# NorthStarUAS/ImageAnalysis

Measured on AMD Instinct MI355X. Metric: image_pairs_matched_per_sec, higher is better.
Workload: dtype u8 (int8 MFMA, int32 accumulate)

## Files before the change

### imageanalysis_amd/csrc/match_knn2sym.hip

```cpp
#include "iamx_common.h"

namespace {

typedef int v4i __attribute__((ext_vector_type(4)));
typedef int v2i __attribute__((ext_vector_type(2)));
typedef int v16i __attribute__((ext_vector_type(16)));
typedef unsigned v2u __attribute__((ext_vector_type(2)));

#ifndef IAMX_DESC_OFFSET
#define IAMX_DESC_OFFSET 128
#endif
constexpr int D = IAMX_DESC_DIM;
constexpr int CHUNK = 128;
constexpr int BIG = 0x3F000000;

struct Pack3Args {
    const void *src;
    const int64_t *src_off;
    int64_t single_n;
    const int32_t *dst_off;
    int8_t *dst;
    int32_t *sn2, *sct, *sperm, *sinv;
    int32_t *n2, *nb, *pos;
    int n_img;
// ... 67 lines not shown
    for (int m = 32; m >= 1; m >>= 1) {
        lo = min(lo, __shfl_xor(lo, m));
        hi = max(hi, __shfl_xor(hi, m));
    }
    if (lane == 0) { atomicMin(&s_lo, lo); atomicMax(&s_hi, hi); }
    __syncthreads();
    lo = s_lo;
    int shift = 0;
    while (((int64_t)s_hi - lo) >> shift >= RANK_BINS) ++shift;
    for (int r = tid; r < n; r += 1024) atomicAdd(&cursor[(key[r] - lo) >> shift], 1);
    __syncthreads();
    int c[4], t = 0, mx = 0;
#pragma unroll
    for (int k = 0; k < 4; ++k) {
        c[k] = cursor[4 * tid + k];
        t += c[k];
        mx = max(mx, c[k]);
    }
    int x = t;
#pragma unroll
    for (int sft = 1; sft < 64; sft <<= 1) {
        const int y = __shfl_up(x, sft);
        if (lane >= sft) x += y;
    }
    if (lane == 63) wsum[wave] = x;
#pragma unroll
    for (int m = 32; m >= 1; m >>= 1) mx = max(mx, __shfl_xor(mx, m));
    if (lane == 0) atomicMax(&s_max, mx);
    __syncthreads();
    int woff = 0;
    for (int w = 0; w < wave; ++w) woff += wsum[w];
    int run = woff + x - t;
#pragma unroll
    for (int k = 0; k < 4; ++k) {
        start[4 * tid + k] = run;
        run += c[k];
    }
    if (tid == 1023) start[RANK_BINS] = run;
    __syncthreads();
    if (s_max > RANK_BIN_LIMIT) {
        if (tid == 0) P.sct[d0] = RANK_TODO;
        return;
    }
    if (tid == 0) P.sct[d0] = 0;
    for (int b = tid; b < RANK_BINS; b += 1024) cursor[b] = start[b];
    __syncthreads();
    for (int r = tid; r < n; r += 1024) {
        const int k = key[r];
        const int at = atomicAdd(&cursor[(k - lo) >> shift], 1);
        list_row[at] = r;
        list_key[at] = k;
    }
    __threadfence_block();
    __syncthreads();
    for (int r = tid; r < n; r += 1024) {
        const int k = key[r], b = (k - lo) >> shift;
        const int e = start[b + 1];
        int cnt = start[b];
        for (int i = start[b]; i < e; ++i) {
            const int kj = list_key[i], j = list_row[i];
            cnt += (kj < k) || (kj == k && j < r);
        }
        P.pos[r0 + r] = cnt;
    }
}

__global__ __launch_bounds__(256) void pack3_rank_kernel(Pack3Args P)
{
    __shared__ __attribute__((aligned(16))) int keys[1024];
    const int img = blockIdx.y;
    const int64_t r0 = P.src_off ? P.src_off[img] : 0;
    const int n = (int)(P.src_off ? P.src_off[img + 1] - r0 : P.single_n);
    if ((int)blockIdx.x * 256 >= n) return;
    if (P.sct[P.dst_off ? P.dst_off[img] : 0] != RANK_TODO) return;
    const int r = blockIdx.x * 256 + threadIdx.x;
    const int mine = r < n ? P.n2[r0 + r] : 0;
    const int tiles = (n + 1023) / 1024, per = (tiles + (int)gridDim.z - 1) / (int)gridDim.z;
    const int b_lo = (int)blockIdx.z * per * 1024, b_hi = min(n, b_lo + per * 1024);
    int cnt = 0;
    for (int base = b_lo; base < b_hi; base += 1024) {
        __syncthreads();
#pragma unroll
        for (int k = 0; k < 4; ++k) {
            const int j = base + k * 256 + threadIdx.x;
            keys[k * 256 + threadIdx.x] = j < n ? P.n2[r0 + j] : 0x7FFFFFFF;
        }
        __syncthreads();
        for (int j = 0; j < 1024; j += 4) {
            const v4i k = *reinterpret_cast<const v4i *>(&keys[j]);
            cnt += (k.x < mine) || (k.x == mine && base + j < r);
            cnt += (k.y < mine) || (k.y == mine && base + j + 1 < r);
            cnt += (k.z < mine) || (k.z == mine && base + j + 2 < r);
            cnt += (k.w < mine) || (k.w == mine && base + j + 3 < r);
        }
    }
    if (r < n) {
        if (gridDim.z == 1) P.pos[r0 + r] = cnt;
        else if (cnt) atomicAdd(&P.pos[r0 + r], cnt);
    }
}

template <typename SRC>
__global__ __launch_bounds__(256) void pack3_scatter_kernel(Pack3Args P)
{
    const int img = blockIdx.y;
    const int64_t r0 = P.src_off ? P.src_off[img] : 0;
    const int n = (int)(P.src_off ? P.src_off[img + 1] - r0 : P.single_n);
    const int d0 = P.dst_off ? P.dst_off[img] : 0;
    const int cap = (n + CHUNK - 1) / CHUNK * CHUNK;
    const int t = blockIdx.x * 256 + threadIdx.x;
    const int r = t >> 3, part = t & 7;
    if (r >= cap) return;
    if (r >= n) {
        *reinterpret_cast<uint4 *>(P.dst + (int64_t)(d0 + r) * D + part * 16) = make_uint4(0, 0, 0, 0);
        if (part == 0) {
            P.sn2[d0 + r] = 0;
            P.sct[d0 + r] = BIG;
            P.sperm[d0 + r] = -1;
            P.sinv[d0 + r] = -1;
        }
        return;
    }
    const SRC *p = static_cast<const SRC *>(P.src) + (r0 + r) * D + part * 16;
    unsigned w[4] = {0, 0, 0, 0};
#pragma unroll
    for (int i = 0; i < 16; ++i)
        w[i >> 2] |= (unsigned)((load_value(p, i) - IAMX_DESC_OFFSET) & 0xFF) << (8 * (i & 3));
    const int pos = d0 + P.pos[r0 + r];
    *reinterpret_cast<uint4 *>(P.dst + (int64_t)pos * D + part * 16) = make_uint4(w[0], w[1], w[2], w[3]);
    if (part == 0) {
        P.sn2[pos] = P.n2[r0 + r];
        P.sct[pos] = P.nb[r0 + r] >> 1;
        P.sperm[pos] = r;
        P.sinv[d0 + r] = pos - d0;
    }
}

constexpr int ROW_NO_BOUND = 0x7F000000;
__device__ __forceinline__ int pack_row_bounds(int L, int U1, int U2)
{
#if defined(IAMX_T_NOPACK)
    return U1;
#else
    typedef unsigned short us2 __attribute__((ext_vector_type(2)));
    const us2 d = __builtin_amdgcn_cvt_pk_u16((unsigned)(U1 - L), (unsigned)(U2 - L));
    return (int)__builtin_bit_cast(unsigned, d);
#endif
}
__device__ __forceinline__ void unpack_row_bounds(v2i e, int &L, int &U1, int &U2)
{
    const int d1 = e.y & 0xFFFF, d2 = (int)((unsigned)e.y >> 16);
    L = e.x;
    U1 = d1 == 0xFFFF ? ROW_NO_BOUND : e.x + d1;
    U2 = d2 == 0xFFFF ? ROW_NO_BOUND : e.x + d2;
}

struct SymArgs {
    const int8_t *sdesc;
    const int32_t *sn2, *sct;
    const int32_t *img_off, *img_n;
    const int32_t *upairs;
    const int32_t *wg_off;
    const int64_t *col_off;
    const int64_t *rowp_off;
    int32_t *col;
    int32_t *rowp;
    int n_u, total_wg;
    uint8_t *colmask;
};

__device__ __forceinline__ int uniform32(int x) { return __builtin_amdgcn_readfirstlane(x); }
__device__ __forceinline__ int64_t uniform64(int64_t x)
{
    return (int64_t)(((uint64_t)(unsigned)__builtin_amdgcn_readfirstlane((int)(x >> 32)) << 32) |
                     (unsigned)__builtin_amdgcn_readfirstlane((int)x));
}

template <bool FUSED>
__device__ __forceinline__ void half_wave_min16(int (&r)[16], int lo, int &m0, int &m1)
{
    int u[4], w[2];
    if constexpr (FUSED) {
        asm("s_nop 1\n\t"
            "v_min_i32_dpp %0, %0, %0 row_ror:8 row_mask:0xf bank_mask:0x3\n\t"
            "v_min_i32_dpp %0, %8, %8 row_ror:8 row_mask:0xf bank_mask:0xc\n\t"
            "v_min_i32_dpp %1, %1, %1 row_ror:8 row_mask:0xf bank_mask:0x3\n\t"
            "v_min_i32_dpp %1, %9, %9 row_ror:8 row_mask:0xf bank_mask:0xc\n\t"
            "v_min_i32_dpp %2, %2, %2 row_ror:8 row_mask:0xf bank_mask:0x3\n\t"
            "v_min_i32_dpp %2, %10, %10 row_ror:8 row_mask:0xf bank_mask:0xc\n\t"
            "v_min_i32_dpp %3, %3, %3 row_ror:8 row_mask:0xf bank_mask:0x3\n\t"
            "v_min_i32_dpp %3, %11, %11 row_ror:8 row_mask:0xf bank_mask:0xc\n\t"
            "v_min_i32_dpp %4, %4, %4 row_ror:8 row_mask:0xf bank_mask:0x3\n\t"
            "v_min_i32_dpp %4, %12, %12 row_ror:8 row_mask:0xf bank_mask:0xc\n\t"
            "v_min_i32_dpp %5, %5, %5 row_ror:8 row_mask:0xf bank_mask:0x3\n\t"
            "v_min_i32_dpp %5, %13, %13 row_ror:8 row_mask:0xf bank_mask:0xc\n\t"
            "v_min_i32_dpp %6, %6, %6 row_ror:8 row_mask:0xf bank_mask:0x3\n\t"
            "v_min_i32_dpp %6, %14, %14 row_ror:8 row_mask:0xf bank_mask:0xc\n\t"
            "v_min_i32_dpp %7, %7, %7 row_ror:8 row_mask:0xf bank_mask:0x3\n\t"
            "v_min_i32_dpp %7, %15, %15 row_ror:8 row_mask:0xf bank_mask:0xc"
            : "+v"(r[0]), "+v"(r[2]), "+v"(r[4]), "+v"(r[6]), "+v"(r[8]), "+v"(r[10]), "+v"(r[12]), "+v"(r[14])
            : "v"(r[1]), "v"(r[3]), "v"(r[5]), "v"(r[7]), "v"(r[9]), "v"(r[11]), "v"(r[13]), "v"(r[15]));
        asm("s_nop 1\n\t"
            "v_min_i32_dpp %0, %0, %0 row_ror:12 row_mask:0xf bank_mask:0x5\n\t"
            "v_min_i32_dpp %0, %4, %4 row_ror:4 row_mask:0xf bank_mask:0xa\n\t"
            "v_min_i32_dpp %1, %1, %1 row_ror:12 row_mask:0xf bank_mask:0x5\n\t"
            "v_min_i32_dpp %1, %5, %5 row_ror:4 row_mask:0xf bank_mask:0xa\n\t"
            "v_min_i32_dpp %2, %2, %2 row_ror:12 row_mask:0xf bank_mask:0x5\n\t"
            "v_min_i32_dpp %2, %6, %6 row_ror:4 row_mask:0xf bank_mask:0xa\n\t"
            "v_min_i32_dpp %3, %3, %3 row_ror:12 row_mask:0xf bank_mask:0x5\n\t"
            "v_min_i32_dpp %3, %7, %7 row_ror:4 row_mask:0xf bank_mask:0xa"
            : "+v"(r[0]), "+v"(r[4]), "+v"(r[8]), "+v"(r[12])
            : "v"(r[2]), "v"(r[6]), "v"(r[10]), "v"(r[14]));
#pragma unroll
        for (int k = 0; k < 4; ++k) u[k] = r[4 * k] + lo;
    } else {
        int s[8];
#pragma unroll
        for (int k = 0; k < 8; ++k) {
            const int a = r[2 * k], b = r[2 * k + 1];
            const int t1 = __builtin_amdgcn_update_dpp(b, a, 0x128, 0xF, 0x3, false);
            const int t2 = __builtin_amdgcn_update_dpp(a, b, 0x128, 0xF, 0xC, false);
            s[k] = min(t1, t2);
        }
#pragma unroll
        for (int k = 0; k < 4; ++k) {
            const int a = s[2 * k], b = s[2 * k + 1];
            const int t1 = __builtin_amdgcn_update_dpp(b, a, 0x12C, 0xF, 0x5, false);
            const int t2 = __builtin_amdgcn_update_dpp(a, b, 0x124, 0xF, 0xA, false);
            u[k] = min(t1, t2) + lo;
        }
    }
#pragma unroll
    for (int k = 0; k < 2; ++k) {
        const v2u x = __builtin_amdgcn_permlane16_swap((unsigned)u[2 * k], (unsigned)u[2 * k + 1], false, false);
        w[k] = min((int)x[0], (int)x[1]);
    }
#pragma unroll
    for (int k = 0; k < 2; ++k) {
        w[k] = min(w[k], __builtin_amdgcn_update_dpp(0, w[k], 0xB1, 0xF, 0xF, true));
        w[k] = min(w[k], __builtin_amdgcn_update_dpp(0, w[k], 0x4E, 0xF, 0xF, true));
    }
    m0 = w[0];
    m1 = w[1];
}

template <int P>
__device__ __forceinline__ void row_min16_piece(int (&r)[16], int (&u)[4], int lo, int *dst)
{
    if constexpr (P == 0) {
        asm("s_nop 1\n\t"
            "v_min_i32_dpp %0, %0, %0 row_ror:8 row_mask:0xf bank_mask:0x3\n\t"
            "v_min_i32_dpp %0, %4, %4 row_ror:8 row_mask:0xf bank_mask:0xc\n\t"
            "v_min_i32_dpp %1, %1, %1 row_ror:8 row_mask:0xf bank_mask:0x3\n\t"
            "v_min_i32_dpp %1, %5, %5 row_ror:8 row_mask:0xf bank_mask:0xc\n\t"
            "v_min_i32_dpp %2, %2, %2 row_ror:8 row_mask:0xf bank_mask:0x3\n\t"
            "v_min_i32_dpp %2, %6, %6 row_ror:8 row_mask:0xf bank_mask:0xc\n\t"
            "v_min_i32_dpp %3, %3, %3 row_ror:8 row_mask:0xf bank_mask:0x3\n\t"
            "v_min_i32_dpp %3, %7, %7 row_ror:8 row_mask:0xf bank_mask:0xc"
            : "+v"(r[0]), "+v"(r[2]), "+v"(r[4]), "+v"(r[6])
            : "v"(r[1]), "v"(r[3]), "v"(r[5]), "v"(r[7]));
    } else if constexpr (P == 1) {
        asm("s_nop 1\n\t"
            "v_min_i32_dpp %0, %0, %0 row_ror:8 row_mask:0xf bank_mask:0x3\n\t"
            "v_min_i32_dpp %0, %4, %4 row_ror:8 row_mask:0xf bank_mask:0xc\n\t"
            "v_min_i32_dpp %1, %1, %1 row_ror:8 row_mask:0xf bank_mask:0x3\n\t"
            "v_min_i32_dpp %1, %5, %5 row_ror:8 row_mask:0xf bank_mask:0xc\n\t"
            "v_min_i32_dpp %2, %2, %2 row_ror:8 row_mask:0xf bank_mask:0x3\n\t"
            "v_min_i32_dpp %2, %6, %6 row_ror:8 row_mask:0xf bank_mask:0xc\n\t"
            "v_min_i32_dpp %3, %3, %3 row_ror:8 row_mask:0xf bank_mask:0x3\n\t"
            "v_min_i32_dpp %3, %7, %7 row_ror:8 row_mask:0xf bank_mask:0xc"
            : "+v"(r[8]), "+v"(r[10]), "+v"(r[12]), "+v"(r[14])
            : "v"(r[9]), "v"(r[11]), "v"(r[13]), "v"(r[15]));
    } else if constexpr (P == 2) {
        asm("s_nop 1\n\t"
            "v_min_i32_dpp %0, %0, %0 row_ror:12 row_mask:0xf bank_mask:0x5\n\t"
            "v_min_i32_dpp %0, %4, %4 row_ror:4 row_mask:0xf bank_mask:0xa\n\t"
            "v_min_i32_dpp %1, %1, %1 row_ror:12 row_mask:0xf bank_mask:0x5\n\t"
            "v_min_i32_dpp %1, %5, %5 row_ror:4 row_mask:0xf bank_mask:0xa\n\t"
            "v_min_i32_dpp %2, %2, %2 row_ror:12 row_mask:0xf bank_mask:0x5\n\t"
            "v_min_i32_dpp %2, %6, %6 row_ror:4 row_mask:0xf bank_mask:0xa\n\t"
            "v_min_i32_dpp %3, %3, %3 row_ror:12 row_mask:0xf bank_mask:0x5\n\t"
            "v_min_i32_dpp %3, %7, %7 row_ror:4 row_mask:0xf bank_mask:0xa"
            : "+v"(r[0]), "+v"(r[4]), "+v"(r[8]), "+v"(r[12])
            : "v"(r[2]), "v"(r[6]), "v"(r[10]), "v"(r[14]));
#pragma unroll
        for (int k = 0; k < 4; ++k) u[k] = r[4 * k] + lo;
    } else {
        int w[2];
#pragma unroll
        for (int k = 0; k < 2; ++k) {
            const v2u x = __builtin_amdgcn_permlane16_swap((unsigned)u[2 * k], (unsigned)u[2 * k + 1], false, false);
            w[k] = min((int)x[0], (int)x[1]);
        }
#pragma unroll
        for (int k = 0; k < 2; ++k) {
            w[k] = min(w[k], __builtin_amdgcn_update_dpp(0, w[k], 0xB1, 0xF, 0xF, true));
            w[k] = min(w[k], __builtin_amdgcn_update_dpp(0, w[k], 0x4E, 0xF, 0xF, true));
        }
        dst[0] = w[0];
        dst[16] = w[1];
    }
}

template <int QW, int NW, int VARIANT, int PIPE, int MERGEW, int SLEEP, bool GROUPLO, int CH, int WPE>
__global__ __launch_bounds__(NW * 64, WPE) void knn2sym_kernel(SymArgs A)
{
    static_assert((VARIANT == 0 || VARIANT == 1) && PIPE > 0 && MERGEW == 2 && SLEEP == 0 && GROUPLO && CH == 128,
                  "only the shipped sweep is implemented");
    constexpr bool ITEMS = VARIANT == 1;
    constexpr int CHUNK = CH;
    constexpr int WGROWS = NW * QW * 32;
    constexpr int NT = NW * 64;
    constexpr int PIECES = CHUNK * D / 16 / NT;
    __shared__ __attribute__((aligned(16))) int8_t lds[2 * CHUNK * D + 2 * CHUNK * 4 + 3 * NW * CHUNK * 4 + 2 * NW * 4 + (2 * NW * CHUNK + NW * 256) * 4];
    int8_t *lds_tile = lds;
    int *lds_tb = reinterpret_cast<int *>(lds + 2 * CHUNK * D);
    int *lds_row = lds_tb + 2 * CHUNK;
    int *lds_cq = lds_row + 3 * NW * CHUNK;
    int *lds_dump = lds_cq + 2 * NW;
    const int tid = threadIdx.x, lane = tid & 63, wave = tid >> 6;
    const int c = lane & 31, g = lane >> 5;

    int vid;
    {
        const int total = A.total_wg, bid = blockIdx.x;
        const int xcd = bid & 7, k = bid >> 3, q = total >> 3, r = total & 7;
        vid = (xcd < r ? xcd * (q + 1) : r * (q + 1) + (xcd - r) * q) + k;
    }
    int lo = 0, hi = A.n_u;
    if constexpr (!ITEMS)
        while (hi - lo > 1) {
            const int mid = (lo + hi) >> 1;
            if (A.wg_off[mid] <= vid) lo = mid; else hi = mid;
        }
    int u = lo, u_end = 0, item_wgi = 0;
    if constexpr (ITEMS) {
        u = A.wg_off[3 * vid];
        u_end = u + A.wg_off[3 * vid + 1];
        item_wgi = A.wg_off[3 * vid + 2];
    }
    v4i bq[QW][4];
    int lo_lane;
    int bimg_held = -1;
    if constexpr (ITEMS) asm volatile("" : "+v"(u_end), "+v"(item_wgi), "+v"(bimg_held));
    int nx_b = 0, nx_a = 0, nx_boff = 0, nx_nb = 0, nx_aoff = 0, nx_na = 0;
    int64_t nx_rowp = 0;
    if constexpr (ITEMS) {
        nx_b = A.upairs[2 * u];
        nx_a = A.upairs[2 * u + 1];
        nx_boff = A.img_off[nx_b];
        nx_nb = A.img_n[nx_b];
        nx_aoff = A.img_off[nx_a];
        nx_na = A.img_n[nx_a];
        nx_rowp = A.rowp_off[u];
    }
    for (;;) {
        const int bimg = ITEMS ? uniform32(nx_b) : A.upairs[2 * u], aimg = ITEMS ? uniform32(nx_a) : A.upairs[2 * u + 1];
        const int boff = ITEMS ? uniform32(nx_boff) : A.img_off[bimg], nb = ITEMS ? uniform32(nx_nb) : A.img_n[bimg];
        const int aoff = ITEMS ? uniform32(nx_aoff) : A.img_off[aimg], na = ITEMS ? uniform32(nx_na) : A.img_n[aimg];
        const int capA = (na + CHUNK - 1) / CHUNK * CHUNK;
        const int nchunks = capA / CHUNK;
        const int wgi = ITEMS ? uniform32(item_wgi) : vid - A.wg_off[u];
        const int q0 = wgi * WGROWS + wave * (QW * 32);
        const bool wave_valid = q0 < nb;
        const int64_t rbase = (ITEMS ? uniform64(nx_rowp) : A.rowp_off[u]) + (int64_t)wgi * capA;
        if constexpr (ITEMS)
            if (uniform32(bimg_held) >= 0) __syncthreads();

        const int rc = (c & 16) | ((c & 3) << 2) | ((c >> 2) & 3);
        if (!ITEMS || bimg != uniform32(bimg_held)) {
            bimg_held = bimg;
#pragma unroll
            for (int qb = 0; qb < QW; ++qb) {
                int row = q0 + QW * rc + qb;
                row = row < nb ? row : nb - 1;
                const v4i *src = reinterpret_cast<const v4i *>(A.sdesc + (int64_t)(boff + row) * D);
#pragma unroll
                for (int s = 0; s < 4; ++s) {
                    bq[qb][s] = ~src[2 * s + g];
                    if constexpr (WPE == 1) asm volatile("" : "+a"(bq[qb][s]));
                }
            }
            lo_lane = 0;
            {
                int spread = 0;
                if (wave_valid) {
                    const int g_lo = rc & ~3, g_hi = rc | 3;
                    const int r_lo = q0 + QW * g_lo < nb ? q0 + QW * g_lo : nb - 1;
                    const int r_hi = q0 + QW * g_hi + QW - 1 < nb ? q0 + QW * g_hi + QW - 1 : nb - 1;
                    lo_lane = A.sn2[boff + r_lo] >> 1;
                    spread = (A.sn2[boff + r_hi] >> 1) - lo_lane;
                }
#pragma unroll
                for (int sh = 32; sh >= 1; sh >>= 1) spread = max(spread, __shfl_xor(spread, sh));
                if (lane == 0) lds_cq[wave] = spread;
            }
        }
        if (!wave_valid) {
#pragma unroll
            for (int k = 0; k < 3 * CHUNK / 64; ++k)
                lds_row[((k / (CHUNK / 64)) * NW + wave) * CHUNK + (k % (CHUNK / 64)) * 64 + lane] = BIG;
        }
        int m[QW][4];
#pragma unroll
        for (int qb = 0; qb < QW; ++qb)
#pragma unroll
            for (int k = 0; k < 4; ++k) m[qb][k] = BIG;

        const int8_t *tbase = A.sdesc + (int64_t)aoff * D;
        const int32_t *tci = A.sct + aoff;
        typedef __attribute__((address_space(3))) void *lds_ptr;
        auto stage_direct = [&](int ch, int buf) {
#pragma unroll
            for (int j = 0; j < PIECES; ++j) {
                const int e = j * NT + tid, row = e >> 3, slot = (e & 7) ^ ((row >> 1) & 7);
                const int8_t *gsrc = tbase + (int64_t)(ch * CHUNK + row) * D + slot * 16;
                int8_t *ldst = lds_tile + buf * (CHUNK * D) + (j * NT + wave * 64) * 16;
                __builtin_amdgcn_global_load_lds(gsrc, (lds_ptr)ldst, 16, 0, 0);
            }
            __builtin_amdgcn_global_load_lds(tci + ch * CHUNK + (tid & (CHUNK - 1)),
                                             (lds_ptr)(lds_tb + buf * CHUNK + (wave & (CHUNK / 64 - 1)) * 64), 4, 0, 0);
        };
        auto wait_direct = [&]() { __builtin_amdgcn_s_waitcnt(0x0F70); };
        constexpr int MROWS = CHUNK / MERGEW;
        static_assert(MROWS == 64 && NW % MERGEW == 0, "one merge row per lane");
        const int mrow = (wave % MERGEW) * MROWS + lane;
        const bool merger = wave < MERGEW;
        constexpr int RSRC_WORD3_DATA_FORMAT_32 = 4 << 15;
        constexpr int RANGE_DROP = 0x7FFFFFF0;
        const __amdgpu_buffer_rsrc_t rowp_rsrc =
            __builtin_amdgcn_make_buffer_rsrc(A.rowp + 2 * rbase, (short)0, capA * 8, RSRC_WORD3_DATA_FORMAT_32);
        int spread_w[NW];
        auto merge_rows = [&](int ch, int rbo, bool store) {
            int L = BIG, U1 = BIG, U2 = BIG;
#pragma unroll
            for (int w = 0; w < NW; ++w) {
                const int R = lds_row[rbo + w * CHUNK + mrow];
                const int lw = R, uw = R + spread_w[w];
                L = min(L, lw);
                U2 = min(max(U1, uw), U2);
                U1 = min(U1, uw);
            }
            __builtin_amdgcn_raw_buffer_store_b64(v2i{L, pack_row_bounds(L, U1, U2)}, rowp_rsrc,
                                                  store ? (ch * CHUNK + mrow) * 8 : RANGE_DROP, 0, 0);
        };

        constexpr int PP = QW / 2, NT4 = CHUNK / 32, NS = NT4 * PP;
        static_assert(NT4 % 2 == 0 && NT4 >= 2, "tile parity must carry across chunks");
        int *const row_dst = (lane & 3) == 0 && wave_valid
            ? lds_row + wave * CHUNK + 8 * ((lane >> 4) & 1) + 4 * g + 2 * ((lane >> 2) & 1) + ((lane >> 3) & 1)
            : lds_dump + wave * 256 + lane;
        v4i aop[2][4], tbop[2][4];
        v16i accs[2][2];
        int r[2][16], bu[4];
#pragma unroll
        for (int k = 0; k < 16; ++k) r[1][k] = BIG;
        auto load_op = [&](int buf, int tile, int k, v4i (&a)[4], v4i (&tbv)[4]) {
            if (k < 4) {
                tbv[k] = *reinterpret_cast<const v4i *>(lds_tb + buf * CHUNK + tile * 32 + 8 * k + 4 * g);
            } else {
                const int s = k - 4, rr = tile * 32 + c, swz = (rr >> 1) & 7;
                a[s] = *reinterpret_cast<const v4i *>(lds_tile + buf * (CHUNK * D) + rr * D + (((2 * s + g) ^ swz) * 16));
            }
        };
        auto issue = [&](int t, int qp, v16i &acc0, v16i &acc1) {
#pragma unroll
            for (int reg = 0; reg < 16; ++reg) acc0[reg] = acc1[reg] = tbop[t & 1][reg >> 2][reg & 3];
#pragma unroll
            for (int s = 0; s < 4; ++s) {
                acc0 = __builtin_amdgcn_mfma_i32_32x32x32_i8(aop[t & 1][s], bq[qp][s], acc0, 0, 0, 0);
                acc1 = __builtin_amdgcn_mfma_i32_32x32x32_i8(aop[t & 1][s], bq[qp + 1][s], acc1, 0, 0, 0);
            }
            if constexpr (WPE == 1) asm volatile("" : "+v"(acc0), "+v"(acc1));
        };

        if constexpr (ITEMS) {
            const int un = u + 1 < u_end ? u + 1 : u;
            nx_b = A.upairs[2 * un];
            nx_a = A.upairs[2 * un + 1];
            nx_rowp = A.rowp_off[un];
        }
        stage_direct(0, 0);
        stage_direct(nchunks > 1 ? 1 : 0, 1);
        wait_direct();
        __syncthreads();
#pragma unroll
        for (int w = 0; w < NW; ++w) spread_w[w] = __builtin_amdgcn_readfirstlane(lds_cq[w]);
        if constexpr (ITEMS) {
            const int b = uniform32(nx_b), a = uniform32(nx_a);
            nx_boff = A.img_off[b];
            nx_nb = A.img_n[b];
            nx_aoff = A.img_off[a];
            nx_na = A.img_n[a];
        }
#pragma unroll
        for (int k = 0; k < 8; ++k) load_op(0, 0, k, aop[0], tbop[0]);
#pragma unroll
        for (int k = 0; k < 8 / PP; ++k) load_op(0, 1, k, aop[1], tbop[1]);
        issue(0, 0, accs[0][0], accs[0][1]);
        __builtin_amdgcn_sched_barrier(0);
        int rbo = 0, rbo_prev = 2 * NW * CHUNK;
        for (int ch = 0; ch < nchunks; ++ch) {
            const int buf = ch & 1;
#pragma unroll
            for (int st = 0; st < NS; ++st) {
                const int t = st / PP, qp = 2 * (st % PP), cur = st & 1;
                if (st == (NT4 - 1) * PP - 1) {
                    __builtin_amdgcn_s_waitcnt(0x0070);
                    __syncthreads();
                    stage_direct(ch + 2 < nchunks ? ch + 2 : nchunks - 1, buf);
                    merge_rows(ch - 1, rbo_prev, merger && ch > 0);
                }
                if (st + 1 < NS) issue((st + 1) / PP, 2 * ((st + 1) % PP), accs[cur ^ 1][0], accs[cur ^ 1][1]);
                else issue(0, 0, accs[cur ^ 1][0], accs[cur ^ 1][1]);
                {
                    const int T = (st + 1) / PP + 1, i = (st + 1) % PP;
#pragma unroll
                    for (int k = i * 8 / PP; k < (i + 1) * 8 / PP; ++k)
                        load_op(T < NT4 ? buf : buf ^ 1, T % NT4, k, aop[T & 1], tbop[T & 1]);
                }
                const v16i acc0 = accs[cur][0], acc1 = accs[cur][1];
                int t0 = min(min(m[qp][t & 3], acc0[0]), acc0[1]);
                int t1m = min(min(m[qp + 1][t & 3], acc1[0]), acc1[1]);
#pragma unroll
                for (int reg = 2; reg < 16; reg += 2) {
                    t0 = min(min(t0, acc0[reg]), acc0[reg + 1]);
                    t1m = min(min(t1m, acc1[reg]), acc1[reg + 1]);
                }
                m[qp][t & 3] = t0;
                m[qp + 1][t & 3] = t1m;
                int (&rc_)[16] = r[t & 1];
                if (qp == 0) {
#pragma unroll
                    for (int reg = 0; reg < 16; ++reg) rc_[reg] = min(acc0[reg], acc1[reg]);
                } else {
#pragma unroll
                    for (int reg = 0; reg < 16; ++reg) rc_[reg] = min(min(rc_[reg], acc0[reg]), acc1[reg]);
                }
                {
                    int (&rp)[16] = r[(t + 1) & 1];
                    const int tp = t > 0 ? t - 1 : NT4 - 1;
                    int *dst = row_dst + (t > 0 ? rbo : rbo_prev) + tp * 32;
                    if constexpr (PP == 1) {
                        int m0, m1;
                        half_wave_min16<true>(rp, lo_lane, m0, m1);
                        dst[0] = m0;
                        dst[16] = m1;
                    } else {
                        if (0 * PP / 4 == st % PP) row_min16_piece<0>(rp, bu, lo_lane, dst);
                        if (1 * PP / 4 == st % PP) row_min16_piece<1>(rp, bu, lo_lane, dst);
                        if (2 * PP / 4 == st % PP) row_min16_piece<2>(rp, bu, lo_lane, dst);
                        if (3 * PP / 4 == st % PP) row_min16_piece<3>(rp, bu, lo_lane, dst);
                    }
                }
#pragma unroll
                for (int i = 0; i < 8; ++i) {
                    __builtin_amdgcn_sched_group_barrier(0x008, 1, 0);
                    __builtin_amdgcn_sched_group_barrier(0x002, PIPE, 0);
                }
                __builtin_amdgcn_sched_barrier(0);
            }
            rbo_prev = rbo;
            rbo = rbo == 2 * NW * CHUNK ? 0 : rbo + NW * CHUNK;
        }
        int64_t col_v = 0;
        if constexpr (ITEMS) col_v = A.col_off[u];
        {
            int m0, m1;
            half_wave_min16<true>(r[(NT4 - 1) & 1], lo_lane, m0, m1);
            int *dst = row_dst + rbo_prev + (NT4 - 1) * 32;
            dst[0] = m0;
            dst[16] = m1;
        }
        wait_direct();
        __syncthreads();
        merge_rows(nchunks - 1, rbo_prev, merger);

        const int64_t col_u = ITEMS ? uniform64(col_v) : 0;
        if (wave_valid) {
            unsigned ownpack = 0;
            int v1s[QW], v2s[QW];
#pragma unroll
            for (int qb = 0; qb < QW; ++qb) {
                const int lo01 = min(m[qb][0], m[qb][1]), hi01 = max(m[qb][0], m[qb][1]);
                const int lo23 = min(m[qb][2], m[qb][3]), hi23 = max(m[qb][2], m[qb][3]);
                const int a1 = min(lo01, lo23), a2 = min(max(lo01, lo23), min(hi01, hi23));
                const int b1 = __shfl_xor(a1, 32), b2 = __shfl_xor(a2, 32);
                const int v1 = min(a1, b1), v2 = min(max(a1, b1), min(a2, b2));
                v1s[qb] = v1;
                v2s[qb] = v2;
#if !defined(IAMX_T_NOMASK)
                const unsigned own = (m[qb][0] <= v2 ? 1u : 0u) | (m[qb][1] <= v2 ? 2u : 0u) |
                                     (m[qb][2] <= v2 ? 4u : 0u) | (m[qb][3] <= v2 ? 8u : 0u);
                ownpack |= own << (4 * qb);
#endif
            }
            const unsigned othpack = A.colmask ? (unsigned)__shfl_xor((int)ownpack, 32) : 0u;
            const int row0 = q0 + QW * rc;
            if (g == 0) {
#pragma unroll
                for (int qb = 0; qb < QW; ++qb)
                    if (row0 + qb < nb)
                        *reinterpret_cast<v2i *>(A.col + 2 * ((ITEMS ? col_u : A.col_off[u]) + row0 + qb)) = v2i{v1s[qb], v2s[qb]};
                if (A.colmask) {
                    uint8_t *dst = A.colmask + (ITEMS ? col_u : A.col_off[u]) + row0;
                    if (QW == 8 && row0 + QW <= nb) {
                        auto spread = [](unsigned nib4) {
                            const unsigned x = (nib4 | (nib4 << 8)) & 0x00FF00FFu;
                            return (x | (x << 4)) & 0x0F0F0F0Fu;
                        };
                        const unsigned lo = spread(ownpack & 0xFFFFu) | (spread(othpack & 0xFFFFu) << 4);
                        const unsigned hi = spread(ownpack >> 16) | (spread(othpack >> 16) << 4);
                        *reinterpret_cast<v2u *>(dst) = v2u{lo, hi};
                    } else {
#pragma unroll
                        for (int qb = 0; qb < QW; ++qb)
                            if (row0 + qb < nb)
                                dst[qb] = (uint8_t)(((ownpack >> (4 * qb)) & 15u) | (((othpack >> (4 * qb)) & 15u) << 4));
                    }
                }
            }
        }
        if constexpr (!ITEMS) break;
        else if (++u == uniform32(u_end)) break;
    }
}

struct NarTask { int p, cls, item0, n; };
struct NarLayout {
    int64_t ctl, pair_base, mask, slot, items, res, tasks, total;
    int64_t item_cap, task_cap;
};
__host__ __device__ inline NarLayout narrow_layout(int64_t rows, int64_t n_pairs)
{
    NarLayout L;
    auto up = [](int64_t v) { return (v + 255) / 256 * 256; };
    L.item_cap = rows;
    L.task_cap = rows / 64 + 80 * n_pairs + 64;
    int64_t o = 0;
    L.ctl = o;        o += 256;
    L.pair_base = o;  o += up(n_pairs * 4);
    L.mask = o;       o += up(rows * 8);
    L.slot = o;       o += up(rows * 8);
    L.items = o;      o += up(L.item_cap * 8);
    L.res = o;        o += up(L.item_cap * 16);
    L.tasks = o;      o += up(L.task_cap * 16);
    L.total = o;
    return L;
}
constexpr int NAR_MIN_TRAIN = 1024;
constexpr int NAR_ITEMS = 256;

struct CandArgs {
    const int32_t *sn2, *sperm, *img_off, *img_n;
    const int32_t *pairs;
    const int32_t *osrc;
    const int32_t *wg_off;
    const int64_t *col_off, *rowp_off, *out_off;
    const int32_t *col, *rowp;
    double thresh;
    uint8_t *keep;
    int32_t *cand_cnt;
    int32_t *cand_q;
    int32_t *task_total;
    int32_t *tasks;
    int32_t *d2;
    int wg_shift;
    const uint8_t *colmask;
    int8_t *nar;
    int64_t rows_total;
    int n_pairs, wgrows;
};

__device__ __forceinline__ void symcand_rows_pair(const CandArgs &A, int p, int pos)
{
    const int qimg = A.pairs[2 * p];
    const int u = A.osrc[2 * p], role = A.osrc[2 * p + 1];
    const int soff = A.img_off[qimg], n = A.img_n[qimg];
    if (pos >= n) return;
    const int cap = (n + CHUNK - 1) / CHUNK * CHUNK;
    const int nwg = A.wg_off[u + 1] - A.wg_off[u];
    const int64_t ob = A.out_off[p];
    const int32_t *rowq = A.rowp + 2 * A.rowp_off[u];
    const int ncls = role == 0 ? 8 : nwg;
    const bool nar_ok = A.nar != nullptr && A.img_n[A.pairs[2 * p + 1]] >= NAR_MIN_TRAIN && ncls <= 64;
    const int n2 = A.sn2[soff + pos], par = n2 & 1;
    long long Lb, Ub;
    int U2 = 0x7FFFFFFF;
    if (role == 0) {
        const v2i v = *reinterpret_cast<const v2i *>(A.col + 2 * (A.col_off[u] + pos));
        const long long cq = n2 >> 1;
        Lb = 2 * (v.x + cq) + par;
        Ub = 2 * (v.y + cq) + par + 1;
    } else {
        int L = 0x7FFFFFFF, U1 = 0x7FFFFFFF;
        for (int w = 0; w < nwg; ++w) {
            int eL, e1, e2;
            unpack_row_bounds(*reinterpret_cast<const v2i *>(rowq + 2 * ((int64_t)w * cap + pos)), eL, e1, e2);
            L = min(L, eL);
            const int n1 = min(U1, e1);
            U2 = min(max(U1, e1), min(U2, e2));
            U1 = n1;
        }
        Lb = 2ll * L + par;
        Ub = 2ll * U2 + par + 1;
    }
    if (Lb < 0) Lb = 0;
    const float f0 = (float)sqrt((double)Lb);
    const float f1 = (float)sqrt((double)Ub);
    const bool k = f1 == 0.0f || (double)f0 * ((double)f0 / (double)f1) < A.thresh;
    const int orig = A.sperm[soff + pos];
    if (k) atomicOr(reinterpret_cast<unsigned *>(A.keep) + ((ob + orig) >> 5), 1u << ((ob + orig) & 31));
    if (k) A.d2[2 * (ob + orig) + 1] = (int)(Ub < 0x7FFFFFFFll ? Ub : 0x7FFFFFFFll);
    if (k && nar_ok) {
        unsigned long long mk = 0ull;
        if (role == 0) {
            mk = A.colmask[A.col_off[u] + pos];
        } else {
            for (int w = 0; w < nwg; ++w)
                if (rowq[2 * ((int64_t)w * cap + pos)] <= U2) mk |= 1ull << w;
        }
        const NarLayout NL = narrow_layout(A.rows_total, A.n_pairs);
        reinterpret_cast<unsigned long long *>(A.nar + NL.mask)[ob + orig] = mk;
    }
}

__global__ __launch_bounds__(256) void symcand_rows_kernel(CandArgs A)
{
    for (int p = blockIdx.y; p < A.n_pairs; p += gridDim.y)
#pragma unroll 1
        for (int k = 0; k < 4; ++k) symcand_rows_pair(A, p, (blockIdx.x * 4 + k) * 256 + threadIdx.x);
}

__global__ __launch_bounds__(256) void symcand_kernel(CandArgs A)
{
    __shared__ int wcnt[4];
    __shared__ int s_base;
    const int p = blockIdx.x;
    const int qimg = A.pairs[2 * p];
    const int u = A.osrc[2 * p], role = A.osrc[2 * p + 1];
    const int n = A.img_n[qimg];
    const int nwg = A.wg_off[u + 1] - A.wg_off[u];
    const int64_t ob = A.out_off[p];
    const NarLayout NL = narrow_layout(A.rows_total, A.n_pairs);
    const int ncls = role == 0 ? 8 : nwg;
    const bool nar_ok = A.nar != nullptr && A.img_n[A.pairs[2 * p + 1]] >= NAR_MIN_TRAIN && ncls <= 64;
    unsigned long long *maskv = reinterpret_cast<unsigned long long *>(A.nar + NL.mask);
    const int lane = threadIdx.x & 63, wave = threadIdx.x >> 6;
    int out = 0;
    for (int base = 0; base < n; base += 256) {
        const int i = base + threadIdx.x;
        const bool k = i < n && ((reinterpret_cast<const unsigned *>(A.keep)[(ob + i) >> 5] >> ((ob + i) & 31)) & 1u);
        const unsigned long long mask = __ballot(k);
        const int before = __popcll(mask & ((1ull << lane) - 1ull));
        if (lane == 0) wcnt[wave] = __popcll(mask);
        __syncthreads();
        int woff = 0, tot = 0;
#pragma unroll
        for (int w = 0; w < 4; ++w) {
            if (w < wave) woff += wcnt[w];
            tot += wcnt[w];
        }
        if (k) A.cand_q[ob + out + woff + before] = i;
        out += tot;
        __syncthreads();
    }
    bool narrow = nar_ok && out > 64;
    if (A.nar != nullptr) {
        __shared__ int cls_cnt[64], cls_off[65], cls_task[65], s_nb;
        int32_t *ctl = reinterpret_cast<int32_t *>(A.nar + NL.ctl);
        int32_t *pair_base = reinterpret_cast<int32_t *>(A.nar + NL.pair_base);
        v2i *slot = reinterpret_cast<v2i *>(A.nar + NL.slot);
        v2i *items = reinterpret_cast<v2i *>(A.nar + NL.items);
        NarTask *ntasks = reinterpret_cast<NarTask *>(A.nar + NL.tasks);
        if (narrow) {
            if (threadIdx.x < 64) cls_cnt[threadIdx.x] = 0;
            __syncthreads();
            int run = 0;
            for (int base = 0; base < out; base += 256) {
                const int i = base + threadIdx.x;
                unsigned long long mk = 0ull;
                if (i < out) mk = maskv[ob + A.cand_q[ob + i]];
                const int nk = __popcll(mk);
                int x = nk;
#pragma unroll
                for (int sft = 1; sft < 64; sft <<= 1) {
                    const int y = __shfl_up(x, sft);
                    if (lane >= sft) x += y;
                }
                if (lane == 63) wcnt[wave] = x;
                __syncthreads();
                int woff = 0, tot = 0;
#pragma unroll
                for (int w = 0; w < 4; ++w) {
                    if (w < wave) woff += wcnt[w];
                    tot += wcnt[w];
                }
                if (i < out) {
                    slot[ob + i] = v2i{run + woff + x - nk, nk};
                    for (unsigned long long b = mk; b; b &= b - 1) atomicAdd(&cls_cnt[__ffsll((long long)b) - 1], 1);
                }
                run += tot;
                __syncthreads();
            }
            if (threadIdx.x == 0) {
                int o = 0, nt = 0;
                for (int cidx = 0; cidx < 64; ++cidx) {
                    cls_off[cidx] = o;
                    cls_task[cidx] = nt;
                    o += cls_cnt[cidx];
                    nt += (cls_cnt[cidx] + NAR_ITEMS - 1) / NAR_ITEMS;
                }
                cls_off[64] = o;
                cls_task[64] = nt;
                const int b0 = atomicAdd(ctl + 1, run);
                bool ok = (int64_t)b0 + run <= NL.item_cap;
                int t0 = 0;
                if (ok) {
                    t0 = atomicAdd(ctl + 0, nt);
                    ok = (int64_t)t0 + nt <= NL.task_cap;
                }
                s_nb = ok ? b0 : -1;
                s_base = t0;
                pair_base[p] = ok ? b0 : -1;
            }
            __syncthreads();
            narrow = s_nb >= 0;
            if (narrow) {
                const int b0 = s_nb, t0 = s_base;
                if (threadIdx.x < 64) {
                    const int cidx = threadIdx.x, cnt_c = cls_cnt[cidx];
                    for (int t = 0; t * NAR_ITEMS < cnt_c; ++t)
                        ntasks[t0 + cls_task[cidx] + t] =
                            NarTask{p, cidx, b0 + cls_off[cidx] + t * NAR_ITEMS, min(NAR_ITEMS, cnt_c - t * NAR_ITEMS)};
                }
                __syncthreads();
                if (threadIdx.x < 64) cls_cnt[threadIdx.x] = 0;
                __syncthreads();
                for (int i = threadIdx.x; i < out; i += 256) {
                    const unsigned long long mk = maskv[ob + A.cand_q[ob + i]];
                    int sl = b0 + slot[ob + i].x;
                    for (unsigned long long b = mk; b; b &= b - 1, ++sl) {
                        const int cidx = __ffsll((long long)b) - 1;
                        const int at = atomicAdd(&cls_cnt[cidx], 1);
                        items[b0 + cls_off[cidx] + at] = v2i{i, sl};
                    }
                }
            }
            __syncthreads();
        } else if (threadIdx.x == 0) {
            pair_base[p] = -1;
        }
    }
    if (narrow) {
        if (threadIdx.x == 0) A.cand_cnt[p] = out;
        return;
    }
    const bool small = out <= 64;
    const int ntask = small ? (out > 0 ? 1 : 0) : (out + (1 << A.wg_shift) - 1) >> A.wg_shift;
    if (threadIdx.x == 0) {
        A.cand_cnt[p] = out;
        s_base = ntask ? atomicAdd(A.task_total + (small ? 0 : 1), ntask) + (small ? 0 : (int)gridDim.x) : 0;
    }
// ... 900 lines not shown
```

Measured before the change: 584,100.

## Hand-schedule PP=4 sweep with inline DPP row minima and interleaved staging

For the PP==4 configuration, the main chunk loop is replaced by a compile-time unrolled sweep. It places row-minimum DPP blocks (inline asm) at computed VALU gap slots between MFMAs and precomputes LDS operand offsets. It also spreads global-to-LDS staging loads and the row merge/store across the stages after the barrier instead of doing them in one burst. The goal is to hide VALU reduction and staging work under MFMA latency with exact sched_group_barrier counts. The hand-tuned gap arithmetic and inline asm add fragility and register pressure, and the other PP values keep the old path.

```diff
diff --git a/imageanalysis_amd/csrc/match_knn2sym.hip b/imageanalysis_amd/csrc/match_knn2sym.hip
--- a/imageanalysis_amd/csrc/match_knn2sym.hip
+++ b/imageanalysis_amd/csrc/match_knn2sym.hip
@@ -393,6 +393,52 @@
     }
 }
 
+template <int P, bool PASS>
+__device__ __forceinline__ void row_min16_block(int (&r)[16], int &after)
+{
+    static_assert(P >= 0 && P < 6, "six blocks");
+    int keep = after;
+    if constexpr (P < 4) {
+        asm("s_nop 1\n\t"
+            "v_min_i32_dpp %0, %0, %0 row_ror:8 row_mask:0xf bank_mask:0x3\n\t"
+            "v_min_i32_dpp %0, %3, %3 row_ror:8 row_mask:0xf bank_mask:0xc\n\t"
+            "v_min_i32_dpp %1, %1, %1 row_ror:8 row_mask:0xf bank_mask:0x3\n\t"
+            "v_min_i32_dpp %1, %4, %4 row_ror:8 row_mask:0xf bank_mask:0xc"
+            : "+v"(r[4 * P]), "+v"(r[4 * P + 2]), "+v"(keep)
+            : "v"(r[4 * P + 1]), "v"(r[4 * P + 3]));
+    } else {
+        constexpr int Q = 8 * (P - 4);
+        asm("s_nop 1\n\t"
+            "v_min_i32_dpp %0, %0, %0 row_ror:12 row_mask:0xf bank_mask:0x5\n\t"
+            "v_min_i32_dpp %0, %3, %3 row_ror:4 row_mask:0xf bank_mask:0xa\n\t"
+            "v_min_i32_dpp %1, %1, %1 row_ror:12 row_mask:0xf bank_mask:0x5\n\t"
+            "v_min_i32_dpp %1, %4, %4 row_ror:4 row_mask:0xf bank_mask:0xa"
+            : "+v"(r[Q]), "+v"(r[Q + 4]), "+v"(keep)
+            : "v"(r[Q + 2]), "v"(r[Q + 6]));
+    }
+    if constexpr (PASS) after = keep;
+}
+
+constexpr int sweep_gap_valu(int nv, int tail, bool blocks, int g)
+{
+    const int last = tail < 6 ? 6 - tail : 0;
+    const int rest = nv - last - (blocks ? 2 : 0), n = blocks ? 5 : 7;
+    if (g == 7) return last;
+    if (blocks && (g == 3 || g == 4)) return 1;
+    const int i = blocks && g > 4 ? g - 2 : g;
+    return rest / n + (i < rest % n ? 1 : 0);
+}
+
+template <int V> struct int_c { static constexpr int value = V; };
+template <int FROM, int TO, typename F>
+__device__ __forceinline__ void static_for(F &&f)
+{
+    if constexpr (FROM < TO) {
+        f(int_c<FROM>{});
+        static_for<FROM + 1, TO>(f);
+    }
+}
+
 template <int QW, int NW, int VARIANT, int PIPE, int MERGEW, int SLEEP, bool GROUPLO, int CH, int WPE>
 __global__ __launch_bounds__(NW * 64, WPE) void knn2sym_kernel(SymArgs A)
 {
@@ -591,8 +637,106 @@
         issue(0, 0, accs[0][0], accs[0][1]);
         __builtin_amdgcn_sched_barrier(0);
         int rbo = 0, rbo_prev = 2 * NW * CHUNK;
+        const int wave_u = uniform32(wave);
+        typedef __attribute__((address_space(3))) const int8_t *lds_bytes;
+        int opoff[4], tboff = 2 * CHUNK * D + 16 * g;
+#pragma unroll
+        for (int s = 0; s < 4; ++s) opoff[s] = c * D + (((2 * s + g) ^ ((c >> 1) & 7)) * 16);
+        auto load_op_at = [&](int tile, int k, v4i (&a)[4], v4i (&tbv)[4]) {
+            if (k < 4) tbv[k] = *reinterpret_cast<const __attribute__((address_space(3))) v4i *>((lds_bytes)lds + tboff + tile * 128 + 32 * k);
+            else a[k - 4] = *reinterpret_cast<const __attribute__((address_space(3))) v4i *>((lds_bytes)lds + opoff[k - 4] + tile * (32 * D));
+        };
+        const unsigned stage_voff = (unsigned)((tid >> 3) * D + (((tid & 7) ^ ((tid >> 4) & 7)) * 16));
+        const unsigned ct_voff = (unsigned)((tid & (CHUNK - 1)) * 4);
         for (int ch = 0; ch < nchunks; ++ch) {
             const int buf = ch & 1;
+            if constexpr (PP == 4) {
+            constexpr int BAR = (NT4 - 1) * PP - 1;
+            static_assert(NW == 4 && PIECES == 4 && BAR + 4 < NS && (NT / 8) % 16 == 0, "the gaps below are form 2's");
+            const int chs = ch + 2 < nchunks ? ch + 2 : nchunks - 1;
+            const int8_t *const sg_tile = tbase + (int64_t)chs * (CHUNK * D);
+            const int8_t *const sg_ct = reinterpret_cast<const int8_t *>(tci + chs * CHUNK);
+            int mR[NW], mL = BIG, mU1 = BIG, mU2 = BIG;
+            static_for<0, NS>([&](auto st_c) {
+                constexpr int st = decltype(st_c)::value;
+                constexpr int t = st / PP, ph = st % PP, qp = 2 * ph, cur = st & 1;
+                constexpr int nst = st + 1 < NS ? st + 1 : 0;
+                if constexpr (st == BAR) {
+                    __builtin_amdgcn_s_waitcnt(0x0070);
+                    __syncthreads();
+                }
+                issue(nst / PP, 2 * (nst % PP), accs[cur ^ 1][0], accs[cur ^ 1][1]);
+                static_for<(st == BAR - 1 ? 1 : 0), (st == BAR - 2 ? 2 : 1)>([&](auto d_c) {
+                    constexpr int sr = st + decltype(d_c)::value;
+                    constexpr int T = (sr + 1) / PP + 1, i = (sr + 1) % PP;
+                    if constexpr (T == NT4 && i == 0) {
+#pragma unroll
+                        for (int s = 0; s < 4; ++s) opoff[s] ^= CHUNK * D;
+                        tboff ^= CHUNK * 4;
+                    }
+#pragma unroll
+                    for (int k = i * 8 / PP; k < (i + 1) * 8 / PP; ++k) load_op_at(T % NT4, k, aop[T & 1], tbop[T & 1]);
+                });
+                constexpr int nv = (ph == 2 ? 36 : ph == 3 ? 40 : 32) + (st == BAR + 2 ? 11 : 0) + (st == BAR + 3 ? 5 : 0) +
+                                   (st >= BAR && st <= BAR + PIECES ? 1 : 0) +
+                                   (st == NS - 1 ? 2 : 0);
+                constexpr int tail = (st == BAR - 1 ? 0 : st == BAR - 2 ? 4 : 2) + (ph == 3 ? 1 + 2 : 0) + (st >= BAR && st <= BAR + PIECES ? 1 : 0) +
+                                     (st == BAR + 1 ? 2 : 0) + (st == BAR + 3 ? 1 : 0);
+                constexpr int blk_at = sweep_gap_valu(nv, tail, true, 0) + sweep_gap_valu(nv, tail, true, 1) +
+                                       sweep_gap_valu(nv, tail, true, 2) - 16;
+                static_assert(ph == 3 || (blk_at >= 0 && blk_at < 15 && blk_at != 7), "gaps 3 and 4 hold two minima of one column chain");
+                const v16i acc0 = accs[cur][0], acc1 = accs[cur][1];
+                int (&rc_)[16] = r[t & 1];
+                int (&rp)[16] = r[(t + 1) & 1];
+#pragma unroll
+                for (int reg = 0; reg < 16; ++reg)
+                    rc_[reg] = qp == 0 ? min(acc0[reg], acc1[reg]) : min(min(rc_[reg], acc0[reg]), acc1[reg]);
+                static_for<0, 16>([&](auto w_c) {
+                    constexpr int w = decltype(w_c)::value;
+                    int &mm = m[qp + (w >> 3)][t & 3];
+                    const v16i &acc = w < 8 ? acc0 : acc1;
+                    mm = min(min(mm, acc[2 * (w & 7)]), acc[2 * (w & 7) + 1]);
+                    if constexpr (ph < 3 && w == blk_at) row_min16_block<2 * ph, true>(rp, mm);
+                    if constexpr (ph < 3 && w == blk_at + 1) row_min16_block<2 * ph + 1, true>(rp, mm);
+                });
+                if constexpr (ph == 2) {
+#pragma unroll
+                    for (int k = 0; k < 4; ++k) bu[k] = rp[4 * k] + lo_lane;
+                }
+                if constexpr (ph == 3) {
+                    int *const dst = row_dst + (t > 0 ? rbo : rbo_prev) + (t > 0 ? t - 1 : NT4 - 1) * 32;
+                    row_min16_piece<3>(rp, bu, lo_lane, dst);
+                }
+                if constexpr (st >= BAR && st < BAR + PIECES)
+                    __builtin_amdgcn_global_load_lds(sg_tile + (st - BAR) * ((NT / 8) * D) + stage_voff,
+                                                     (lds_ptr)(lds_tile + buf * (CHUNK * D) + ((st - BAR) * NT + wave_u * 64) * 16), 16, 0, 0);
+                if constexpr (st == BAR + PIECES)
+                    __builtin_amdgcn_global_load_lds(sg_ct + ct_voff,
+                                                     (lds_ptr)(lds_tb + buf * CHUNK + (wave_u & (CHUNK / 64 - 1)) * 64), 4, 0, 0);
+                if constexpr (st == BAR + 1) {
+#pragma unroll
+                    for (int w = 0; w < NW; ++w) mR[w] = lds_row[rbo_prev + w * CHUNK + mrow];
+                }
+                if constexpr (st == BAR + 2) {
+#pragma unroll
+                    for (int w = 0; w < NW; ++w) {
+                        const int uw = mR[w] + spread_w[w];
+                        mL = min(mL, mR[w]);
+                        mU2 = min(max(mU1, uw), mU2);
+                        mU1 = min(mU1, uw);
+                    }
+                }
+                if constexpr (st == BAR + 3)
+                    __builtin_amdgcn_raw_buffer_store_b64(v2i{mL, pack_row_bounds(mL, mU1, mU2)}, rowp_rsrc,
+                                                          merger && ch > 0 ? ((ch - 1) * CHUNK + mrow) * 8 : RANGE_DROP, 0, 0);
+                static_for<0, 8>([&](auto g_c) {
+                    constexpr int g = decltype(g_c)::value;
+                    __builtin_amdgcn_sched_group_barrier(0x008, 1, 0);
+                    __builtin_amdgcn_sched_group_barrier(0x002, sweep_gap_valu(nv, tail, ph < 3, g) + (g == 7 ? 3 : 0), 0);
+                });
+                __builtin_amdgcn_sched_barrier(0);
+            });
+            } else {
 #pragma unroll
             for (int st = 0; st < NS; ++st) {
                 const int t = st / PP, qp = 2 * (st % PP), cur = st & 1;
@@ -650,6 +794,7 @@
                     __builtin_amdgcn_sched_group_barrier(0x002, PIPE, 0);
                 }
                 __builtin_amdgcn_sched_barrier(0);
+            }
             }
             rbo_prev = rbo;
             rbo = rbo == 2 * NW * CHUNK ? 0 : rbo + NW * CHUNK;
```

New measurement: 608,500 (median of 6 runs). 1.04x the previous value.
